# longkaimao/Sentinel

Measured on AMD Instinct MI355X. Metric: flow decisions/sec (node) at 1M flowIds, 1/2/4/8 GPU; HBM GB/s vs peak, higher is better.
Workload: dtype int64; 1 GPU; C3 cluster token server: ClusterFlowChecker, FLOW_THRESHOLD_GLOBAL, S=10/1000 ms; flow_ids=1000000, flow_ids_per_gpu=1000000, parallelism=hash-sharded flowIds x1, rollup=none (1 GPU), namespace_limiter=off

## Files before the change

sentinel_amd/csrc/engine.h:

```cpp
#pragma once

#include <hip/hip_runtime.h>
#include <stddef.h>
#include <stdint.h>

#include "../../include/sentinel_gpu.h"
#include "search_dev.h"

namespace sg {

struct alignas(16) Rule {
    double thr;
    double isec;
    int32_t S;
    int32_t wl;
    int32_t wl_idx;
    int32_t wait_ms;
};
static_assert(sizeof(Rule) == 32, "Rule layout");

struct alignas(64) Bucket {
    int64_t start;
    int64_t c[SG_NUM_EVENTS];
};
static_assert(sizeof(Bucket) == 64, "Bucket layout");

struct alignas(16) BucketHot {
    int64_t start;
    int32_t pass;
    int32_t wait;
};
static_assert(sizeof(BucketHot) == 16, "BucketHot layout");

__device__ __forceinline__ void store_hot(BucketHot* h, int64_t start, int64_t pass, int64_t wait) {
    BucketHot x;
    x.start = start;
    x.pass = (int32_t)pass;
    x.wait = (int32_t)wait;
    *h = x;
}

struct alignas(16) Occ {
    int64_t pass;
    int64_t pass_req;
};

#ifndef SG_SORT_ROUNDS
#define SG_SORT_ROUNDS 16
#endif
constexpr int kSortRounds = SG_SORT_ROUNDS;
constexpr int kMaxWl = 8;
constexpr uint32_t kMaxPeriods = 1u << 16;
constexpr int kShortMax = 256;
constexpr int kLdsBnd = 4096;
constexpr int kLdsBndFlow = 1024;
#ifndef SG_RECW
#define SG_RECW 32
#endif
constexpr int kRecW = SG_RECW;
constexpr int kClasses = 6;
constexpr uint32_t kClassMax[kClasses - 1] = {4, 16, 64, 256, 1024};

constexpr int kErrTime = 1;
constexpr int kErrPeriods = 2;
constexpr int kErrInternal = 16;
constexpr int kErrExchange = 64;

struct BatchArgs {
    const sg_req* req;
    sg_result* out;
    uint64_t n;
    uint64_t* rec;
    uint32_t* hist0;
    uint32_t* csum0;
    int hist0_bits;
    uint64_t* rec_sorted;
    int kshift;
    int abits;
    uint64_t imask;
    uint64_t amask;
    uint64_t aesc;
    uint32_t K;
    const Rule* rules;
    Bucket* ring;
    BucketHot* hot;
    Occ* occ;
    int stride;
    double max_occ_ratio;
    int n_wl;
    int32_t wl[kMaxWl];
    uint32_t* bnd;
    int64_t* p0;
    uint32_t* np;
    int* err;
    int64_t* last_ts;
    int check_last;
    int64_t* front_ts;
    int walk_cus;
    uint32_t* long_list;
    uint32_t* long_count;
    uint32_t* short_list;
    uint32_t* short_count;
    uint32_t* short_key;
    uint32_t* long_key;
    uint32_t* seg_end;
    uint32_t* seg_start;
    uint32_t* short_end;
    uint32_t* long_end;
    int seg_marked;
    uint32_t* long_pend;
    uint64_t class_off[kClasses];
    uint32_t short_max;
    uint32_t* exit_cnt;
    uint64_t exit_amask;
    int dbg;
    int narrow;
    int generic_walker;
    int tiny;
    unsigned long long* dbg_ctr;
    uint4* skips;
    uint32_t* skip_count;
    uint32_t skip_cap;
    int hist0_shift;
    int bin_on;
    int prep_tiles;
    int bin_dshift;
    int bin_bsh;
    uint32_t bin_R;
    uint2* hot_tab;
    uint32_t* hot_key;
    uint64_t* bin_buf;
    const uint32_t* bin_tot;
};

constexpr int kBinDigit = 10;
constexpr uint32_t kBinRegular = 512;
constexpr uint32_t kBinHot = (1u << kBinDigit) - kBinRegular - 1;
constexpr uint32_t kBinDrop = (1u << kBinDigit) - 1;
constexpr int kBinMaxBsh = 11;
constexpr int kHotBucketBits = 9;
constexpr uint32_t kHotWays = 4;
constexpr uint32_t kHotTab = kHotWays << kHotBucketBits;
constexpr uint32_t kHotEmpty = 0xFFFFFFFFu;
__host__ __device__ __forceinline__ uint32_t hot_hash(uint32_t key) {
    return (key * 2654435761u) >> (32 - kHotBucketBits);
}

constexpr int kLongPeriods = 16;
constexpr uint32_t kLongTab = 65536;
constexpr uint32_t kSkipMin = 256;
constexpr uint32_t kSkipPiece = 4096;

constexpr int kMaxLim = 8;
constexpr int kLimSamples = 10;
constexpr int kLimWindowMs = 100;

struct LimRing {
    int64_t start[kLimSamples];
    int64_t count[kLimSamples];
};

static_assert(sizeof(sg_req) % sizeof(int64_t) == 0 && sizeof(sg_cparam_req) % sizeof(int64_t) == 0 &&
                  offsetof(sg_req, ts_ms) == 0 && offsetof(sg_cparam_req, ts_ms) == 0,
              "LimArgs::ts strides over the request records");
struct LimArgs {
    int n_lim;
    int wl_idx;
    double qps[kMaxLim];
    const uint8_t* rule_lim;
    uint8_t* slot;
    uint32_t* tile_tot;
    uint32_t* tile_off;
    uint32_t* arrivals;
    uint32_t* prefix;
    uint32_t* quota;
    LimRing* ring;
    const uint32_t* xg;
    const int64_t* ts;
    uint32_t ts_stride;
    int64_t t_base;
    uint32_t n_ms;
    int world, rank;
};

hipError_t launch_limiter(const BatchArgs& a, const LimArgs& L, hipStream_t stream);
hipError_t launch_limiter_plan_only(const BatchArgs& a, const LimArgs& L, hipStream_t stream);
hipError_t launch_lim_arrivals(const sg_req* req, uint64_t n, uint32_t K, const uint8_t* rule_lim, int64_t t_base,
                               uint32_t n_ms, uint32_t* counts, int* err, hipStream_t stream);
hipError_t launch_lim_arrivals_param(const sg_cparam_req* req, uint64_t n, uint32_t K, const uint8_t* rule_lim,
                                     int64_t t_base, uint32_t n_ms, uint32_t* counts, int* err, hipStream_t stream);

constexpr int kErrNonPositive = 4;
constexpr int kErrTableFull = 8;

struct PRule {
    int64_t token_count;
    int64_t duration_sec;
    int32_t burst;
    int32_t behavior;
    int32_t max_queueing_ms;
    uint32_t hot_begin, hot_count;
    uint32_t pad;
    uint64_t table_base;
    uint64_t table_mask;
};

struct alignas(16) CxSide {
    int64_t t;
    uint32_t psl;
    uint32_t node;
};

struct alignas(32) PSlot {
    uint64_t value;
    uint32_t flags;
    uint32_t pad;
    int64_t time;
    int64_t tokens;
};

constexpr uint32_t kPcBuckets = 2048;

struct PArgs {
    const sg_param_req* req;
    int32_t* out;
    uint64_t n;
    uint64_t* rec;
    uint64_t* rec_sorted;
    int ibits;
    uint64_t imask;
    int gshift;
    uint32_t* msb;
    int64_t* mt0;
    uint32_t* mnp;
    uint16_t* mbk;
    int bshift;
    const PRule* rules;
    uint32_t n_rules;
    const sg_param_hot_item* hot;
    PSlot* table;
    uint64_t total_slots;
    int* err;
    int64_t* last_ts;
    uint32_t* long_list;
    uint32_t* long_count;
    uint32_t short_max;
};

struct alignas(32) PSThread {
    unsigned long long owner;
    uint64_t value;
    int64_t count;
    int64_t pad;
};

hipError_t launch_param_clear(PSlot* table, uint64_t n, hipStream_t stream);
hipError_t launch_param_batch(const PArgs& p, const BatchArgs& sg, uint64_t* a_buf, uint64_t* b_buf, uint32_t* hist,
                              int lo_bit, int hi_bit, uint64_t** sorted_out, hipStream_t stream, hipStream_t aux,
                              hipEvent_t fork, hipEvent_t join);

struct PaceRule {
    double count;
    int32_t max_queueing_ms;
    int32_t pad;
};

struct PaceArgs {
    const sg_pace_req* req;
    int32_t* out;
    uint64_t n;
    uint64_t* rec;
    uint64_t* rec_sorted;
    int ibits;
    uint64_t imask;
    const PaceRule* rules;
    uint32_t n_rules;
    int64_t* latest;
    int* err;
    int64_t* last_ts;
    uint32_t* long_list;
    uint32_t* long_count;
    uint32_t* short_list;
    uint32_t short_max;
    int gshift;
    uint32_t* msb;
    int64_t* mt0;
    uint32_t* mnp;
    uint16_t* mbk;
    int bshift;
    uint64_t class_off[kClasses];
};

hipError_t launch_pace_batch(const PaceArgs& p, uint64_t* a_buf, uint64_t* b_buf, uint32_t* hist, int lo_bit, int hi_bit,
                             uint64_t** sorted_out, hipStream_t stream, hipStream_t aux, hipEvent_t fork,
                             hipEvent_t join);

constexpr int kErrBounds = 32;

struct CPRule {
    double count;
    double isec;
    int32_t S;
    int32_t wl;
    int32_t global;
    int32_t connected;
    uint32_t hot_begin, hot_count;
    uint64_t table_base;
    uint64_t table_mask;
    int32_t wl_idx;
    int32_t pad;
};

struct CPBucket {
    int64_t start;
    int64_t count;
};

struct CPArgs {
    const sg_cparam_req* req;
    const uint64_t* values;
    uint64_t n_values;
    sg_result* out;
    uint64_t n;
    uint64_t* rec;
    int ibits;
    uint64_t imask;
    const CPRule* rules;
    uint32_t n_rules;
    const sg_param_hot_item* hot;
    uint64_t* keys;
    CPBucket* ring;
    int stride;
    uint64_t total_slots;
    uint64_t per;
    int* err;
    int64_t* last_ts;
};

struct CPBatch {
    uint32_t* owner;
    uint8_t* chk;
    uint8_t* assume;
    uint64_t* rec;
    int pbits;
    uint64_t pmask;
    int idbits;
    uint64_t idmask;
    int n_wl;
    int32_t wl[kMaxWl];
    uint32_t* bnd;
    int64_t* p0;
    uint32_t* np;
    int* changed;
    const int* changed_prev;
    CPBucket* save;
    uint32_t* pslot;
    uint32_t* dflag;
    uint32_t* item_start;
    uint32_t* item_end;
    uint32_t* item_slot;
    uint32_t* slot_item;
    uint32_t* din;
    uint32_t* din_count;
    uint32_t* dout;
// ... 574 lines not shown
```

sentinel_amd/csrc/engine.hip:

```cpp
#include "engine.h"

#include <algorithm>
#include <cstdlib>
#include <mutex>

namespace sg {


__device__ __forceinline__ int32_t java_d2i(double x) {
    if (x != x) return 0;
    if (x >= 2147483647.0) return INT32_MAX;
    if (x <= -2147483648.0) return INT32_MIN;
    return (int32_t)x;
}

__device__ __forceinline__ int lane_id() { return (int)__lane_id(); }

__device__ __forceinline__ double qps_of(int64_t sum, double isec) { return avg_div((double)sum, isec); }

__device__ __forceinline__ int64_t wave_sum(int64_t v) {
#pragma unroll
    for (int o = 32; o > 0; o >>= 1) v += __shfl_xor((long long)v, o, 64);
    return v;
}
// ... 1050 lines not shown
    __syncthreads();
    if (diag) tk1 = __builtin_amdgcn_s_memrealtime();
    uint32_t tk[kBinPer], sst[kBinPer], slot[kBinPer], gb = 0;
    if (small) {
        const Cnt16 cnt{lw};
#pragma unroll
        for (int u = 0; u < kBinRows; ++u) {
            const uint32_t j = c0 + (uint32_t)u * 64 + (uint32_t)lane;
            if (j < c1) cnt.inc((uint32_t)wave * kBinKeys + (uint32_t)(v[u] >> a.kshift) - kb0);
        }
        __syncthreads();
        if (diag) tk2 = __builtin_amdgcn_s_memrealtime();
        bin_scan_lists(a, cnt, nk, wsum, lcnt, tk, sst, slot);
        __syncthreads();
        if (tid < kL && lcnt[tid]) gb = atomicAdd(tid == kClasses ? a.long_count : a.short_count + tid, lcnt[tid]);
        if (diag) tk3 = __builtin_amdgcn_s_memrealtime();
        uint32_t pos[kBinRows / 2];
#pragma unroll
        for (int u = 0; u < kBinRows; ++u) {
            const uint32_t j = c0 + (uint32_t)u * 64 + (uint32_t)lane;
            const bool valid = j < c1;
            const uint32_t d = valid ? (uint32_t)(v[u] >> a.kshift) - kb0 : 0u;
            const uint64_t peers = match_key(d) & __ballot(valid);
            const uint32_t ci = (uint32_t)wave * kBinKeys + d;
            const uint32_t c = cnt.get(ci);
            const uint32_t p16 = valid ? c + (uint32_t)__popcll(peers & lt) : 0xFFFFu;
            pos[u / 2] = (u & 1) ? (pos[u / 2] | (p16 << 16)) : p16;
            cnt.set(ci, c + (uint32_t)__popcll(peers));
            __builtin_amdgcn_sched_barrier(0);
        }
        if (diag) tp4 = __builtin_amdgcn_s_memrealtime();
        uint64_t* stage = lds + (kBinWaves * kBinKeys * 2) / 8;
        uint64_t* dst = a.rec_sorted + s0;
        for (uint32_t w0 = 0; w0 < len; w0 += kBinStage) {
#pragma unroll
            for (int u = 0; u < kBinRows; ++u) {
                const uint32_t p = (pos[u / 2] >> ((u & 1) * 16)) & 0xFFFFu;
                if (p != 0xFFFFu && p - w0 < kBinStage) stage[p - w0] = v[u];
            }
            __syncthreads();
            const uint32_t m = min(kBinStage, len - w0);
            for (uint32_t p = tid; p < m; p += kBinThreads) dst[w0 + p] = stage[p];
            __syncthreads();
        }
    } else {
        uint32_t(*cnt)[kBinKeys] = reinterpret_cast<uint32_t(*)[kBinKeys]>(lw);
        struct Cnt32 {
            uint32_t* w;
            __device__ __forceinline__ uint32_t get(uint32_t i) const { return w[i]; }
            __device__ __forceinline__ void set(uint32_t i, uint32_t x) const { w[i] = x; }
        } c32{lw};
        for (uint32_t r0 = c0; r0 < c1; r0 += 64u * kBinRows) {
            if (r0 != c0) {
#pragma unroll
                for (int u = 0; u < kBinRows; ++u) v[u] = src[min(r0 + (uint32_t)u * 64 + (uint32_t)lane, last)];
            }
#pragma unroll
            for (int u = 0; u < kBinRows; ++u) {
                const uint32_t j = r0 + (uint32_t)u * 64 + (uint32_t)lane;
                if (j < c1) atomicAdd(&cnt[wave][(uint32_t)(v[u] >> a.kshift) - kb0], 1u);
            }
        }
        __syncthreads();
        if (diag) tk2 = __builtin_amdgcn_s_memrealtime();
        bin_scan_lists(a, c32, nk, wsum, lcnt, tk, sst, slot);
        __syncthreads();
        if (tid < kL && lcnt[tid]) gb = atomicAdd(tid == kClasses ? a.long_count : a.short_count + tid, lcnt[tid]);
        if (diag) tk3 = __builtin_amdgcn_s_memrealtime();
        uint64_t* dst = a.rec_sorted + s0;
        for (uint32_t r0 = c0; r0 < c1; r0 += 64u * kBinRows) {
#pragma unroll
            for (int u = 0; u < kBinRows; ++u) v[u] = src[min(r0 + (uint32_t)u * 64 + (uint32_t)lane, last)];
#pragma unroll
            for (int u = 0; u < kBinRows; ++u) {
                const uint32_t j = r0 + (uint32_t)u * 64 + (uint32_t)lane;
                const bool valid = j < c1;
                const uint32_t d = valid ? (uint32_t)(v[u] >> a.kshift) - kb0 : 0u;
                const uint64_t peers = match_key(d) & __ballot(valid);
                const uint32_t c = cnt[wave][d];
                if (valid) {
                    dst[c + (uint32_t)__popcll(peers & lt)] = v[u];
                    if (lane == __builtin_ctzll(peers)) cnt[wave][d] = c + (uint32_t)__popcll(peers);
                }
                __builtin_amdgcn_sched_barrier(0);
            }
        }
    }
    if (diag) tp5 = __builtin_amdgcn_s_memrealtime();
    if (tid < kL) lbase[tid] = gb;
    __syncthreads();
    if (diag) tp6 = __builtin_amdgcn_s_memrealtime();
    bin_emit(a, lbase, s0, kb0, tk, sst, slot);
    if (diag) {
        __syncthreads();
        if (tid == 0) {
            const uint64_t tk4 = __builtin_amdgcn_s_memrealtime();
            if (small) {
                atomicAdd(&a.dbg_ctr[48], (unsigned long long)(tp4 - tk3));
                atomicAdd(&a.dbg_ctr[49], (unsigned long long)(tp5 - tp4));
                atomicAdd(&a.dbg_ctr[50], (unsigned long long)(tp6 - tp5));
                atomicAdd(&a.dbg_ctr[51], (unsigned long long)(tk4 - tp6));
            }
            atomicAdd(&a.dbg_ctr[40], (unsigned long long)(tk1 - tk0));
            atomicAdd(&a.dbg_ctr[41], (unsigned long long)(tk2 - tk1));
            atomicAdd(&a.dbg_ctr[42], (unsigned long long)(tk3 - tk2));
            atomicAdd(&a.dbg_ctr[43], (unsigned long long)(tk4 - tk3));
            atomicAdd(&a.dbg_ctr[44], 1ull);
            atomicAdd(&a.dbg_ctr[45], small ? 0ull : 1ull);
            atomicAdd(&a.dbg_ctr[47], (unsigned long long)len);
        }
    }
}

__global__ void __launch_bounds__(1024) k_hot_update(BatchArgs a) {
    __shared__ uint32_t hcnt[32];
    __shared__ uint32_t thr, nslot;
    __shared__ uint32_t tkey[kHotTab], tslot[kHotTab], bfill[kHotTab / kHotWays];
    const uint32_t tid = threadIdx.x;
    if (tid < 32) hcnt[tid] = 0;
    if (tid == 0) nslot = 0;
    for (uint32_t x = tid; x < kHotTab; x += 1024) {
        tkey[x] = kHotEmpty;
        tslot[x] = 0;
    }
    for (uint32_t x = tid; x < kHotTab / kHotWays; x += 1024) bfill[x] = 0;
    __syncthreads();
    const uint32_t nl = *a.err ? 0u : *a.long_count;
    for (uint32_t i = tid; i < nl; i += 1024) {
        const uint32_t len = a.long_end[i] - a.long_list[i];
        atomicAdd(&hcnt[31 - __clz(len)], 1u);
    }
    __syncthreads();
    if (tid == 0) {
        uint32_t cum = 0, t = 0;
        for (int c = 31; c >= 0; --c) {
            cum += hcnt[c];
            if (cum >= kBinHot) {
                t = (uint32_t)c;
                break;
            }
        }
        thr = t;
    }
    __syncthreads();
    for (int pass = 0; pass < 2; ++pass) {
        for (uint32_t i = tid; i < nl; i += 1024) {
            const uint32_t len = a.long_end[i] - a.long_list[i];
            const uint32_t c = 31 - __clz(len);
            if (pass == 0 ? c <= thr : c != thr) continue;
            if (nslot >= kBinHot) continue;
            const uint32_t k = a.long_key[i];
            const uint32_t bk = hot_hash(k);
            const uint32_t w = atomicAdd(&bfill[bk], 1u);
            if (w >= kHotWays) continue;
            const uint32_t s = atomicAdd(&nslot, 1u);
            if (s >= kBinHot) {
                tkey[bk * kHotWays + w] = kHotEmpty;
                continue;
            }
            a.hot_key[s] = k;
            tkey[bk * kHotWays + w] = k;
            tslot[bk * kHotWays + w] = s;
        }
        __syncthreads();
    }
    for (uint32_t x = tid; x < kHotTab; x += 1024) a.hot_tab[x] = make_uint2(tkey[x], tslot[x]);
}

__global__ void __launch_bounds__(256) k_hot_reset(uint2* hot_tab) {
    for (uint32_t x = threadIdx.x; x < kHotTab; x += 256) hot_tab[x] = make_uint2(kHotEmpty, 0u);
}

__device__ __forceinline__ void stage_periods(const BatchArgs& a) {
    uint32_t tot = 0;
    for (int w = 0; w < a.n_wl; ++w) tot += a.np[w];
    const bool lds = tot <= (uint32_t)kLdsBndFlow && !(a.dbg & 1);
    uint32_t off = 0;
    for (int w = 0; w < a.n_wl; ++w) {
        const uint32_t npw = a.np[w];
        if (lds) {
            const uint32_t* g = a.bnd + (size_t)w * kMaxPeriods;
            for (uint32_t i = threadIdx.x; i < npw; i += blockDim.x) g_sbnd[off + i] = g[i];
        }
        if (threadIdx.x == 0) g_boff[w] = off;
        off += npw;
    }
    if (threadIdx.x == 0) g_blds = lds ? 1 : 0;
    if (threadIdx.x < (unsigned)a.n_wl) {
        g_p0[threadIdx.x] = a.p0[threadIdx.x];
        g_np[threadIdx.x] = a.np[threadIdx.x];
    }
    for (uint32_t x = threadIdx.x; x < (uint32_t)a.n_wl * (kModS + 1); x += blockDim.x) {
        const uint32_t w = x / (kModS + 1), m = x % (kModS + 1);
        g_p0mod[w][m] = m ? (uint8_t)(a.p0[w] % (int64_t)m) : (uint8_t)0;
    }
    __syncthreads();
}

template <bool L>
__device__ __forceinline__ void walk_long_body(const BatchArgs& a) {
    const int lane = lane_id();
    const uint32_t n_long = *a.long_count;
    const uint32_t wave = blockIdx.x * (blockDim.x / 64) + threadIdx.x / 64;
    const uint32_t nwaves = gridDim.x * (blockDim.x / 64);
    for (uint32_t item = wave; item < n_long; item += nwaves) {
        const uint64_t s = a.long_list[item];
        uint32_t k;
        uint64_t e;
        if (a.long_key && a.seg_end) {
            k = a.long_key[item];
            e = a.long_end ? a.long_end[item] : a.seg_end[k];
        } else {
            k = (uint32_t)(a.rec_sorted[s] >> a.kshift);
            e = gallop_search(s + (a.short_max ? a.short_max : 1), a.n, [&](uint64_t p) {
                return (uint32_t)(a.rec_sorted[p] >> a.kshift) != k;
            }, lane);
        }
        const uint64_t t0 = (a.dbg & 64) ? __builtin_amdgcn_s_memrealtime() : 0;
        walk_wave<L>(a, k, s, e, item);
        if (a.dbg & 64) {
            const uint64_t t1 = __builtin_amdgcn_s_memrealtime();
            const uint64_t len = e - s;
            const int b = len <= 64 ? 0 : len <= 256 ? 1 : len <= 1024 ? 2 : 3;
            if (lane == 0) {
                atomicAdd(&a.dbg_ctr[16 + 2 * b], 1ull);
                atomicAdd(&a.dbg_ctr[17 + 2 * b], (unsigned long long)(t1 - t0));
                atomicMax(&a.dbg_ctr[24 + b], (unsigned long long)(t1 - t0));
            }
        }
    }
}

__global__ void __launch_bounds__(256) k_long_bounds(BatchArgs a) {
    if (*a.err) return;
    const uint32_t n_long = min(*a.long_count, kLongTab);
    const uint32_t total = n_long * (uint32_t)kLongPeriods;
    for (uint32_t t = blockIdx.x * blockDim.x + threadIdx.x; t < total; t += gridDim.x * blockDim.x) {
        const uint32_t item = t / kLongPeriods, q = t % kLongPeriods;
        const uint32_t k = a.long_key[item];
        const int w = a.rules[k].wl_idx;
        const uint32_t npw = a.np[w];
        if (npw > (uint32_t)kLongPeriods || q + 1 >= npw) continue;
        const uint32_t nb = a.bnd[(size_t)w * kMaxPeriods + q + 1];
        uint64_t lo = a.long_list[item], hi = a.long_end ? a.long_end[item] : a.seg_end[k];
        while (lo < hi) {
            const uint64_t mid = (lo + hi) >> 1;
            if ((uint32_t)((a.rec_sorted[mid] >> a.abits) & a.imask) >= nb) hi = mid;
            else lo = mid + 1;
        }
        a.long_pend[t] = (uint32_t)lo;
    }
}

#ifndef SG_WLONG_BLOCKS
#define SG_WLONG_BLOCKS 2
#endif
__global__ void __launch_bounds__(256, SG_WLONG_BLOCKS) k_walk_long(BatchArgs a) {
    if (*a.err || (a.dbg & 4096)) return;
    stage_periods(a);
    if (g_blds) walk_long_body<true>(a);
    else walk_long_body<false>(a);
}


struct SlotSnap {
    int32_t st, pass, wait;
};
constexpr int32_t kSnapOld = -(1 << 30);

__device__ __forceinline__ int32_t rel32(int64_t x) {
    return x > (int64_t)INT32_MAX ? INT32_MAX : x < (int64_t)INT32_MIN ? INT32_MIN : (int32_t)x;
}

__device__ __forceinline__ int32_t snap_rel(int64_t start, int64_t T0) {
    if (start == INT64_MIN) return INT32_MIN;
    const int64_t d = start - T0;
    return d < (int64_t)kSnapOld ? kSnapOld : d > (int64_t)(1 << 30) ? (1 << 30) : (int32_t)d;
}

__device__ __forceinline__ bool narrow_span(const BatchArgs& a, int64_t T0) {
    bool ok = true;
    for (int w = 0; w < a.n_wl; ++w) {
        const int64_t wl = a.wl[w];
        const int64_t b = a.p0[w] * wl;
        ok = ok && (b + ((int64_t)a.np[w] + 1) * wl - T0 < (1ll << 29)) &&
             (b - ((int64_t)a.stride + 1) * wl - T0 > -(1ll << 29));
    }
    return ok;
}

__device__ __forceinline__ bool tiny_active(const BatchArgs& a) {
    return a.tiny && a.narrow && narrow_span(a, a.p0[0] * (int64_t)a.wl[0]);
}

__device__ __forceinline__ void store_bucket(Bucket* b, BucketHot* h, int64_t start, const int64_t* c) {
    ulonglong2* p = reinterpret_cast<ulonglong2*>(b);
    p[0] = make_ulonglong2((unsigned long long)start, (unsigned long long)c[0]);
    p[1] = make_ulonglong2((unsigned long long)c[1], (unsigned long long)c[2]);
    p[2] = make_ulonglong2((unsigned long long)c[3], (unsigned long long)c[4]);
    p[3] = make_ulonglong2((unsigned long long)c[5], (unsigned long long)c[6]);
    store_hot(h, start, c[SG_EV_PASS], c[SG_EV_WAITING]);
}

constexpr int kBlk = 4;

template <int SM, bool L>
__device__ __forceinline__ void walk_reg(const BatchArgs& a, bool act, uint32_t k, uint64_t s, uint64_t e,
                                         const Rule& R, const Occ& occ, SlotSnap* snap, uint64_t* buf, int64_t T0) {
    Bucket* ring = a.ring + (size_t)k * a.stride;
    BucketHot* hot = a.hot + (size_t)k * a.stride;
    const int S = R.S;
    const int64_t wl = R.wl;
    PeriodCursor<L> pc;
    pc.init(a, act ? R.wl_idx : 0);
    const int64_t P0 = g_p0[act ? R.wl_idx : 0];
    PeriodState ps;
    ps.occ_pass = occ.pass;
    ps.occ_req = occ.pass_req;
#pragma unroll
    for (int ev = 0; ev < SG_NUM_EVENTS; ++ev) ps.cur[ev] = 0;
    ps.wo_pass = ps.wo_wait = ps.head_other = 0;
    int I = -1;
    int64_t ws = 0;
    const uint64_t n1 = a.n - 1;
    uint64_t nb[kBlk];
    uint64_t p = s;
    int left = kBlk;
    bool more = act && p + kBlk < e;
#pragma unroll
    for (int u = 0; u < kBlk; ++u) nb[u] = a.rec_sorted[min(p + kBlk + u, n1)];
    bool live = act;
    uint32_t qn = 0;
    Decoded dn;
    auto peek = [&]() {
        if (p + (uint64_t)(kBlk - left) >= e) {
            live = false;
            return;
        }
        dn = decode(a, buf[0]);
        qn = pc.of(dn.idx);
    };
    auto advance = [&]() {
#pragma unroll
        for (int v = 0; v < kBlk - 1; ++v) buf[v] = buf[v + 1];
        buf[kBlk - 1] = ~0ull;
        if (--left == 0) {
            if (!more) {
                live = false;
                return;
            }
#pragma unroll
            for (int u = 0; u < kBlk; ++u) buf[u] = nb[u];
            p += kBlk;
            left = kBlk;
            more = p + kBlk < e;
#pragma unroll
            for (int u = 0; u < kBlk; ++u) nb[u] = a.rec_sorted[min(p + kBlk + u, n1)];
        }
    };
    if (live) peek();
    while (__ballot(live)) {
        if (live && qn != pc.q) {
            if (I >= 0) {
                if (!(a.dbg & 512)) store_bucket(ring + I, hot + I, ws, ps.cur);
                snap[I].st = (int32_t)(ws - T0);
                snap[I].pass = (int32_t)ps.cur[SG_EV_PASS];
                snap[I].wait = (int32_t)ps.cur[SG_EV_WAITING];
            }
            const uint32_t qprev = pc.q;
            pc.seek(qn);
            const int64_t P = P0 + (int64_t)qn;
            I = I < 0 ? period_slot(R.wl_idx, qn, S) : (int)((uint32_t)(I + (int)(qn - qprev)) % (uint32_t)S);
            ws = P * wl;
            const int64_t lo_rel = ws - (int64_t)S * wl - T0;
            const int32_t lo32 = rel32(lo_rel);
            const int h = I + 1 == S ? 0 : I + 1;
            int32_t sx[SM], px[SM], wx[SM];
#pragma unroll
            for (int x = 0; x < SM; ++x) {
                sx[x] = snap[x].st;
                px[x] = snap[x].pass;
                wx[x] = snap[x].wait;
            }
            uint32_t wp = 0, ww = 0, ho = 0;
#pragma unroll
            for (int x = 0; x < SM; ++x) {
                const bool v = (x < S) & (x != I) & (sx[x] > lo32);
                const uint32_t m = v ? 0xFFFFFFFFu : 0u;
                wp += (uint32_t)px[x] & m;
                ww += (uint32_t)wx[x] & m;
                ho = (x == h) ? ((uint32_t)px[x] & m) : ho;
            }
            ps.wo_pass = (int64_t)wp;
            ps.wo_wait = (int64_t)ww;
            ps.head_other = (int64_t)ho;
            const int32_t stI_rel = snap[I].st;
            const int64_t stI = stI_rel == INT32_MIN ? INT64_MIN : T0 + (int64_t)stI_rel;
            int64_t cI[SG_NUM_EVENTS];
            if (stI == ws) {
#pragma unroll
                for (int ev = 0; ev < SG_NUM_EVENTS; ++ev) cI[ev] = ring[I].c[ev];
            }
            open_bucket(ps, stI, cI, ws);
        }
        while (live && qn == pc.q) {
            const double latest = qps_of(ps.wo_pass + ps.cur[SG_EV_PASS], R.isec);
            const double next_remaining = R.thr - latest - (double)dn.acq;
            if (next_remaining >= 0) {
                ps.cur[SG_EV_PASS] += dn.acq;
                ps.cur[SG_EV_PASS_REQUEST] += 1;
                if (dn.prio) ps.cur[SG_EV_OCCUPIED_PASS] += dn.acq;
                if (!(a.dbg & 256)) store_result(a.out, dn.idx, SG_STATUS_OK, java_d2i(next_remaining), 0);
            } else {
                int32_t wait;
                const int32_t stt = decide_fail(R, a.max_occ_ratio, ps, dn.acq, dn.prio, &wait);
                if (stt != SG_STATUS_BLOCKED && !(a.dbg & 256)) store_result(a.out, dn.idx, stt, 0, wait);
            }
            advance();
            if (live) peek();
        }
    }

    if (act) {
        if (I >= 0) store_bucket(ring + I, hot + I, ws, ps.cur);
        if (ps.occ_pass != occ.pass || ps.occ_req != occ.pass_req) {
            Occ o;
            o.pass = ps.occ_pass;
            o.pass_req = ps.occ_req;
            a.occ[k] = o;
        }
    }
}

__device__ __forceinline__ void wait_vm0() { __builtin_amdgcn_s_waitcnt(0x0F70); }

template <int R>
__device__ __forceinline__ void glds_rows(const uint32_t* src, uint32_t* wrecs) {
    if constexpr (R > 0) {
        glds_rows<R - 1>(src, wrecs);
        __builtin_amdgcn_global_load_lds((const __attribute__((address_space(1))) void*)src,
                                         (__attribute__((address_space(3))) void*)(wrecs + (R - 1) * 64 - 2 * (R - 1)),
                                         4, 8 * (R - 1), 0);
    }
}

template <int R>
__device__ __forceinline__ void stage_records(const BatchArgs& a, uint32_t* wrecs, uint64_t p) {
    glds_rows<R>(reinterpret_cast<const uint32_t*>(a.rec_sorted + p), wrecs);
}

template <int SM, bool L>
__device__ __forceinline__ void walk_lds(const BatchArgs& a, bool act, uint32_t k, uint64_t s, uint64_t e,
                                         const Rule& R, const Occ& occ, SlotSnap* snap, uint32_t* wrecs, int lane,
                                         int64_t T0, int rows) {
    Bucket* ring = a.ring + (size_t)k * a.stride;
    BucketHot* hot = a.hot + (size_t)k * a.stride;
    const int S = R.S;
    const int64_t wl = R.wl;
    PeriodCursor<L> pc;
    pc.init(a, act ? R.wl_idx : 0);
    const int64_t P0 = g_p0[act ? R.wl_idx : 0];
    PeriodState ps;
    ps.occ_pass = occ.pass;
    ps.occ_req = occ.pass_req;
#pragma unroll
    for (int ev = 0; ev < SG_NUM_EVENTS; ++ev) ps.cur[ev] = 0;
    ps.wo_pass = ps.wo_wait = ps.head_other = 0;
    int I = -1;
    int64_t ws = 0;
    uint64_t wb = s;
    uint64_t p = s;
    bool live = act && p < e;
    bool park = false;
    uint32_t win = (uint32_t)rows;
    uint32_t qn = 0;
    Decoded dn;
    auto peek = [&]() {
        if (p >= e) {
            live = false;
            return;
        }
        if (p - wb >= (uint64_t)win) {
            park = true;
            return;
        }
        dn = decode_c(a, wrecs[(uint32_t)(p - wb) * 64 + lane]);
        qn = pc.of(dn.idx);
    };
    if (live) peek();
    for (;;) {
        if (!__ballot(live && !park)) {
            if (!__ballot(live)) break;
            if (park) {
                stage_records<kRecW>(a, wrecs, p);
                wb = p;
                win = kRecW;
            }
            wait_vm0();
            __builtin_amdgcn_wave_barrier();
            if (park) {
                park = false;
                peek();
            }
            continue;
        }
        if (live && !park && qn != pc.q) {
            if (I >= 0) {
                store_bucket(ring + I, hot + I, ws, ps.cur);
                snap[I].st = (int32_t)(ws - T0);
                snap[I].pass = (int32_t)ps.cur[SG_EV_PASS];
                snap[I].wait = (int32_t)ps.cur[SG_EV_WAITING];
            }
            const uint32_t qprev = pc.q;
            pc.seek(qn);
            const int64_t P = P0 + (int64_t)qn;
            I = I < 0 ? period_slot(R.wl_idx, qn, S) : (int)((uint32_t)(I + (int)(qn - qprev)) % (uint32_t)S);
            ws = P * wl;
            const int64_t lo_rel = ws - (int64_t)S * wl - T0;
            const int32_t lo32 = rel32(lo_rel);
            const int h = I + 1 == S ? 0 : I + 1;
            int32_t sx[SM], px[SM], wx[SM];
#pragma unroll
            for (int x = 0; x < SM; ++x) {
                sx[x] = snap[x].st;
                px[x] = snap[x].pass;
                wx[x] = snap[x].wait;
            }
            uint32_t wp = 0, ww = 0, ho = 0;
#pragma unroll
            for (int x = 0; x < SM; ++x) {
                const bool v = (x < S) & (x != I) & (sx[x] > lo32);
                const uint32_t m = v ? 0xFFFFFFFFu : 0u;
                wp += (uint32_t)px[x] & m;
                ww += (uint32_t)wx[x] & m;
                ho = (x == h) ? ((uint32_t)px[x] & m) : ho;
            }
            ps.wo_pass = (int64_t)wp;
            ps.wo_wait = (int64_t)ww;
            ps.head_other = (int64_t)ho;
            const int32_t stI_rel = snap[I].st;
            const int64_t stI = stI_rel == INT32_MIN ? INT64_MIN : T0 + (int64_t)stI_rel;
            int64_t cI[SG_NUM_EVENTS];
            if (stI == ws) {
#pragma unroll
                for (int ev = 0; ev < SG_NUM_EVENTS; ++ev) cI[ev] = ring[I].c[ev];
            }
            open_bucket(ps, stI, cI, ws);
        }
        while (live && !park && qn == pc.q) {
            const double latest = qps_of(ps.wo_pass + ps.cur[SG_EV_PASS], R.isec);
            const double next_remaining = R.thr - latest - (double)dn.acq;
            if (next_remaining >= 0) {
                ps.cur[SG_EV_PASS] += dn.acq;
                ps.cur[SG_EV_PASS_REQUEST] += 1;
                if (dn.prio) ps.cur[SG_EV_OCCUPIED_PASS] += dn.acq;
                store_result(a.out, dn.idx, SG_STATUS_OK, java_d2i(next_remaining), 0);
            } else {
                int32_t wait;
                const int32_t stt = decide_fail(R, a.max_occ_ratio, ps, dn.acq, dn.prio, &wait);
                if (stt != SG_STATUS_BLOCKED) store_result(a.out, dn.idx, stt, 0, wait);
            }
            ++p;
            peek();
        }
    }
    if (act) {
        if (I >= 0) store_bucket(ring + I, hot + I, ws, ps.cur);
        if (ps.occ_pass != occ.pass || ps.occ_req != occ.pass_req) {
            Occ o;
            o.pass = ps.occ_pass;
            o.pass_req = ps.occ_req;
            a.occ[k] = o;
        }
    }
}

constexpr int kGatherMaxS = 10;
#ifndef SG_SHORT_BLOCKS
#define SG_SHORT_BLOCKS 3
#endif
constexpr int kShortBlocksPerCu = SG_SHORT_BLOCKS;

template <int SM, bool L>
__device__ __forceinline__ void walk_short_lds(const BatchArgs& a, SlotSnap* snap_all, uint32_t* recs_all) {
    static_assert(SM > 0, "LDS ring snapshot");
    const int lane = lane_id();
    const bool tiny = tiny_active(a);
    SlotSnap* snap = snap_all + (threadIdx.x / 64) * (64 * SM);
    uint32_t* wrecs = recs_all + (threadIdx.x / 64) * (kRecW * 64);
    uint32_t cnt[kClasses], grp_end[kClasses];
    uint32_t total = 0;
#pragma unroll
    for (int c = kClasses - 1; c >= 0; --c) {
        cnt[c] = (c == 0 && tiny) ? 0u : a.short_count[c];
        total += (cnt[c] + 63) / 64;
        grp_end[c] = total;
    }
    const uint32_t wave = blockIdx.x * (blockDim.x / 64) + threadIdx.x / 64;
    const uint32_t nwaves = gridDim.x * (blockDim.x / 64);
    if (wave >= total) return;
    const int64_t T0 = a.p0[0] * (int64_t)a.wl[0];
    auto desc = [&](uint32_t g, int& c, bool& act, uint32_t& s, uint32_t& k, uint32_t& e) {
        c = kClasses - 1;
        uint32_t g0 = 0;
        while (g >= grp_end[c]) {
            g0 = grp_end[c];
            --c;
        }
        c = __builtin_amdgcn_readfirstlane(c);
        const uint32_t i = (g - g0) * 64 + (uint32_t)lane;
        act = i < cnt[c];
        const uint64_t li = a.class_off[c] + (act ? i : 0u);
        s = a.short_list[li];
        k = a.short_key[li];
        e = a.short_end[li];
    };
    int c_n;
    bool act_n;
    uint32_t s_n, k_n, e_n;
    desc(wave, c_n, act_n, s_n, k_n, e_n);
    for (uint32_t g = wave; g < total; g += nwaves) {
        const uint64_t tw0 = (a.dbg & 64) ? __builtin_amdgcn_s_memrealtime() : 0;
        const int c = c_n;
        const bool act = act_n;
        const uint64_t s = s_n;
        const uint32_t k = k_n;
        const uint64_t e = e_n;
        const Rule R = a.rules[k];
        const Occ occ = a.occ[k];
        static_assert(kRecW >= (int)kClassMax[1], "the first window of class 1 must fit the lane's LDS rows");
        const int rows = c == 0 ? (int)kClassMax[0] : c == 1 ? (int)kClassMax[1] : kRecW;
        if (c == 0) stage_records<kClassMax[0]>(a, wrecs, s);
        else if (c == 1) stage_records<kClassMax[1]>(a, wrecs, s);
        else stage_records<kRecW>(a, wrecs, s);
        desc(min(g + nwaves, total - 1), c_n, act_n, s_n, k_n, e_n);
        {
            constexpr int kT = SM;
            int gl = lane;
            asm volatile("" : "+v"(gl));
            ulonglong2 v[kT];
#pragma unroll
            for (int t = 0; t < kT; ++t) {
                const int pc = t * 64 + gl;
                const int j = pc / kT;
                const int q = pc % kT;
                const uint32_t kj = (uint32_t)__shfl((int)k, j, 64);
                const int qq = q < a.stride ? q : 0;
                v[t] = *reinterpret_cast<const ulonglong2*>(a.hot + (size_t)kj * a.stride + qq);
            }
            __builtin_amdgcn_sched_barrier(0);
#pragma unroll
            for (int t = 0; t < kT; ++t) asm volatile("" ::"v"(v[t].x), "v"(v[t].y));
#pragma unroll
            for (int t = 0; t < kT; ++t) {
                const int pc = t * 64 + gl;
                SlotSnap& d = snap[pc];
                d.st = snap_rel((int64_t)v[t].x, T0);
                d.pass = (int32_t)(uint32_t)v[t].y;
                d.wait = (int32_t)(uint32_t)(v[t].y >> 32);
            }
        }
        wait_vm0();
        __builtin_amdgcn_fence(__ATOMIC_RELEASE, "wavefront");
        __builtin_amdgcn_wave_barrier();
        __builtin_amdgcn_fence(__ATOMIC_ACQUIRE, "wavefront");
        const uint64_t tw1 = (a.dbg & 64) ? __builtin_amdgcn_s_memrealtime() : 0;
        walk_lds<SM, L>(a, act, k, s, e, R, occ, snap + lane * SM, wrecs, lane, T0, rows);
        if (a.dbg & 64) {
            const uint64_t tw2 = __builtin_amdgcn_s_memrealtime();
            if (lane == 0) {
                atomicAdd(&a.dbg_ctr[0], (unsigned long long)(tw2 - tw0));
                atomicAdd(&a.dbg_ctr[1 + c], 1ull);
                atomicAdd(&a.dbg_ctr[7 + c], (unsigned long long)(tw1 - tw0));
                atomicAdd(&a.dbg_ctr[7 + c], (unsigned long long)(tw2 - tw1) << 32);
            }
        }
    }
}

template <int SM, bool L, bool C>
__device__ __forceinline__ void walk_short_body(const BatchArgs& a, SlotSnap* snap_all, uint32_t* recs_all) {
    if constexpr (SM > 0 && C) {
        const int64_t T0 = a.p0[0] * (int64_t)a.wl[0];
        if (a.narrow && narrow_span(a, T0)) {
            walk_short_lds<SM, L>(a, snap_all, recs_all);
            return;
        }
    }
    constexpr int kSnapPerWave = SM > 0 ? 64 * SM : 1;
    const int lane = lane_id();
    const bool tiny = tiny_active(a);
    SlotSnap* snap = snap_all + (threadIdx.x / 64) * kSnapPerWave;
    uint32_t cnt[kClasses], grp_end[kClasses];
    uint32_t total = 0;
#pragma unroll
    for (int c = kClasses - 1; c >= 0; --c) {
        cnt[c] = (c == 0 && tiny) ? 0u : a.short_count[c];
        total += (cnt[c] + 63) / 64;
        grp_end[c] = total;
    }
    const uint32_t wave = blockIdx.x * (blockDim.x / 64) + threadIdx.x / 64;
    const uint32_t nwaves = gridDim.x * (blockDim.x / 64);
    const int64_t T0 = a.p0[0] * (int64_t)a.wl[0];
    const bool snap_ok = SM > 0 && a.narrow && narrow_span(a, T0);
    for (uint32_t g = wave; g < total; g += nwaves) {
        int c = kClasses - 1;
        uint32_t g0 = 0;
        while (g >= grp_end[c]) {
            g0 = grp_end[c];
            --c;
        }
        c = __builtin_amdgcn_readfirstlane(c);
        const uint32_t i = (g - g0) * 64 + (uint32_t)lane;
        const bool act = i < cnt[c];
        if constexpr (SM > 0 && !C) if (snap_ok) {
            const uint64_t tw0 = (a.dbg & 64) ? __builtin_amdgcn_s_memrealtime() : 0;
            const uint64_t li = a.class_off[c] + (act ? i : 0u);
            const uint64_t s = a.short_list[li];
            const uint32_t k = a.short_key[li];
            const uint64_t e = a.short_end ? a.short_end[li] : a.seg_end[k];
            const Rule R = a.rules[k];
            const Occ occ = a.occ[k];
            uint64_t buf[kBlk];
#pragma unroll
            for (int u = 0; u < kBlk; ++u) buf[u] = a.rec_sorted[min(s + u, a.n - 1)];
            {
                constexpr int kT = SM;
                int gl = lane;
                asm volatile("" : "+v"(gl));
                {
                    ulonglong2 v[SM];
#pragma unroll
                    for (int t = 0; t < SM; ++t) {
                        const int pc = t * 64 + gl;
                        const int j = pc / kT;
                        const int q = pc % kT;
                        const uint32_t kj = (uint32_t)__shfl((int)k, j, 64);
                        const int qq = q < a.stride ? q : 0;
                        v[t] = *reinterpret_cast<const ulonglong2*>(a.hot + (size_t)kj * a.stride + qq);
                    }
#pragma unroll
                    for (int t = 0; t < SM; ++t) {
                        SlotSnap& d = snap[t * 64 + gl];
                        d.st = snap_rel((int64_t)v[t].x, T0);
                        d.pass = (int32_t)(uint32_t)v[t].y;
                        d.wait = (int32_t)(uint32_t)(v[t].y >> 32);
                    }
                }
                __builtin_amdgcn_fence(__ATOMIC_RELEASE, "wavefront");
                __builtin_amdgcn_wave_barrier();
                __builtin_amdgcn_fence(__ATOMIC_ACQUIRE, "wavefront");
            }
            const uint64_t tw1 = (a.dbg & 64) ? __builtin_amdgcn_s_memrealtime() : 0;
            walk_reg<SM, L>(a, act, k, s, e, R, occ, snap + lane * SM, buf, T0);
            if (a.dbg & 64) {
                const uint64_t tw2 = __builtin_amdgcn_s_memrealtime();
                if (lane == 0) {
                    atomicAdd(&a.dbg_ctr[0], (unsigned long long)(tw2 - tw0));
                    atomicAdd(&a.dbg_ctr[1 + c], 1ull);
                    atomicAdd(&a.dbg_ctr[7 + c], (unsigned long long)(tw1 - tw0));
                    atomicAdd(&a.dbg_ctr[7 + c], (unsigned long long)(tw2 - tw1) << 32);
                }
            }
            continue;
        }
        if (!act) continue;
        const uint64_t s = a.short_list[a.class_off[c] + i];
        const uint32_t k = (uint32_t)(a.rec_sorted[s] >> a.kshift);
        const uint64_t lim = s + (uint64_t)min(a.short_max, c < kClasses - 1 ? kClassMax[c] : 0xFFFFFFFFu) + 1;
        uint64_t e = s + 1;
        while (e < a.n && e < lim && (uint32_t)(a.rec_sorted[e] >> a.kshift) == k) ++e;
        walk_serial<L>(a, k, s, e);
    }
}

template <int SM, bool C>
#ifndef SG_SHORT_C_BLOCKS
#define SG_SHORT_C_BLOCKS 2
#endif
__global__ void __launch_bounds__(256, C ? SG_SHORT_C_BLOCKS : kShortBlocksPerCu) k_walk_short(BatchArgs a) {
    static_assert(SM <= kGatherMaxS, "LDS budget of the ring snapshot");
    __shared__ SlotSnap snap_all[4 * (SM > 0 ? 64 * SM : 1)];
    __shared__ uint32_t recs_all[SM > 0 && C ? 4 * kRecW * 64 : 1];
    if (*a.err || (a.dbg & 8192)) return;
    stage_periods(a);
    if (g_blds) walk_short_body<SM, true, C>(a, snap_all, recs_all);
    else walk_short_body<SM, false, C>(a, snap_all, recs_all);
}

template <int SM, bool L>
__device__ __forceinline__ void walk_tiny_body(const BatchArgs& a) {
    constexpr int kR = (int)kClassMax[0];
    const uint32_t cnt = a.short_count[0];
    const uint64_t base = a.class_off[0];
    const int64_t T0 = a.p0[0] * (int64_t)a.wl[0];
    for (uint32_t t = blockIdx.x * blockDim.x + threadIdx.x; t < cnt; t += gridDim.x * blockDim.x) {
        const uint64_t s = a.short_list[base + t];
        const uint32_t k = a.short_key[base + t];
        const uint32_t e = a.short_end[base + t];
        const Rule R = a.rules[k];
        const Occ occ = a.occ[k];
        uint64_t r0 = a.rec_sorted[s], r1 = a.rec_sorted[min(s + 1, a.n - 1)];
        uint64_t r2 = a.rec_sorted[min(s + 2, a.n - 1)], r3 = a.rec_sorted[min(s + 3, a.n - 1)];
        static_assert(kR == 4, "four record registers");
        Bucket* ring = a.ring + (size_t)k * a.stride;
        BucketHot* hot = a.hot + (size_t)k * a.stride;
        int32_t st[SM], pa[SM], wa[SM];
#pragma unroll
        for (int x = 0; x < SM; ++x) {
            const int xx = x < R.S ? x : 0;
            const ulonglong2 hv = *reinterpret_cast<const ulonglong2*>(hot + xx);
            st[x] = snap_rel((int64_t)hv.x, T0);
            pa[x] = (int32_t)(uint32_t)hv.y;
            wa[x] = (int32_t)(uint32_t)(hv.y >> 32);
        }
        PeriodCursor<L> pc;
        pc.init(a, R.wl_idx);
        const int64_t P0 = g_p0[R.wl_idx];
        const int S = R.S;
        PeriodState ps;
        ps.occ_pass = occ.pass;
        ps.occ_req = occ.pass_req;
#pragma unroll
        for (int ev = 0; ev < SG_NUM_EVENTS; ++ev) ps.cur[ev] = 0;
        ps.wo_pass = ps.wo_wait = ps.head_other = 0;
        int I = -1;
        int64_t ws = 0;
        const uint32_t m = e - (uint32_t)s;
        for (uint32_t u = 0; u < m; ++u) {
            const Decoded d = decode(a, r0);
            r0 = r1;
            r1 = r2;
            r2 = r3;
            const uint32_t q = pc.of(d.idx);
            if (q != pc.q) {
                if (I >= 0) {
                    store_bucket(ring + I, hot + I, ws, ps.cur);
#pragma unroll
                    for (int x = 0; x < SM; ++x) {
                        st[x] = x == I ? (int32_t)(ws - T0) : st[x];
                        pa[x] = x == I ? (int32_t)ps.cur[SG_EV_PASS] : pa[x];
                        wa[x] = x == I ? (int32_t)ps.cur[SG_EV_WAITING] : wa[x];
                    }
                }
                const uint32_t qprev = pc.q;
                pc.seek(q);
                const int64_t P = P0 + (int64_t)q;
                I = I < 0 ? period_slot(R.wl_idx, q, S) : (int)((uint32_t)(I + (int)(q - qprev)) % (uint32_t)S);
                ws = P * R.wl;
                const int64_t lo_rel = ws - (int64_t)S * R.wl - T0;
                const int32_t lo32 = rel32(lo_rel);
                const int h = I + 1 == S ? 0 : I + 1;
                uint32_t wp = 0, ww = 0, ho = 0;
                int32_t stI_rel = INT32_MIN;
#pragma unroll
                for (int x = 0; x < SM; ++x) {
                    const bool v = (x < S) & (x != I) & (st[x] > lo32);
                    const uint32_t mk = v ? 0xFFFFFFFFu : 0u;
                    wp += (uint32_t)pa[x] & mk;
                    ww += (uint32_t)wa[x] & mk;
                    ho = (x == h) ? ((uint32_t)pa[x] & mk) : ho;
                    stI_rel = x == I ? st[x] : stI_rel;
                }
                ps.wo_pass = (int64_t)wp;
                ps.wo_wait = (int64_t)ww;
                ps.head_other = (int64_t)ho;
                const int64_t stI = stI_rel == INT32_MIN ? INT64_MIN : T0 + (int64_t)stI_rel;
                int64_t cI[SG_NUM_EVENTS];
// ... 379 lines not shown
```

Measured before the change: 22.40 billion decisions/s.

## Fast-path blocked records once a period is saturated

Adds a saturation flag per period: once a request fails and even an acquire of one would exceed the threshold, later non-priority requests below the escalation bound are counted as blocked without the floating-point QPS check or the decide_fail call. In the LDS window walker, runs of up to kSatN plain records are checked and accumulated into the block counters in one step. The goal is to cut per-record work in hot, over-limit flows. It relies on the packed record-code bit layout and adds optional debug counters.

```diff
diff --git a/sentinel_amd/csrc/engine.h b/sentinel_amd/csrc/engine.h
--- a/sentinel_amd/csrc/engine.h
+++ b/sentinel_amd/csrc/engine.h
@@ -60,6 +60,8 @@
 constexpr int kRecW = SG_RECW;
 constexpr int kClasses = 6;
 constexpr uint32_t kClassMax[kClasses - 1] = {4, 16, 64, 256, 1024};
+constexpr int kDbgSatRecords = 14;
+constexpr int kDbgSatRuns = 15;
 
 constexpr int kErrTime = 1;
 constexpr int kErrPeriods = 2;
diff --git a/sentinel_amd/csrc/engine.hip b/sentinel_amd/csrc/engine.hip
--- a/sentinel_amd/csrc/engine.hip
+++ b/sentinel_amd/csrc/engine.hip
@@ -1376,6 +1376,25 @@
     store_hot(h, start, c[SG_EV_PASS], c[SG_EV_WAITING]);
 }
 
+__device__ __forceinline__ bool period_saturated(double thr, double latest) { return !(thr - latest - 1.0 >= 0); }
+
+#ifndef SG_SAT_N
+#define SG_SAT_N 8
+#endif
+constexpr int kSatN = SG_SAT_N;
+
+__device__ __forceinline__ bool sat_plain(uint32_t c, uint32_t next_b) {
+    return ((c >> 8) < next_b) & ((c & 1u) == 0u) & ((c & 0xFEu) != 0xFEu);
+}
+
+__device__ __forceinline__ void sat_counters(const BatchArgs& a, uint32_t rec, uint32_t ent, int lane) {
+    const int64_t r = wave_sum((int64_t)rec), n = wave_sum((int64_t)ent);
+    if (lane == 0 && r) {
+        atomicAdd(&a.dbg_ctr[kDbgSatRecords], (unsigned long long)r);
+        atomicAdd(&a.dbg_ctr[kDbgSatRuns], (unsigned long long)n);
+    }
+}
+
 constexpr int kBlk = 4;
 
 template <int SM, bool L>
@@ -1406,6 +1425,8 @@
     bool live = act;
     uint32_t qn = 0;
     Decoded dn;
+    bool sat = false;
+    bool run = false;
     auto peek = [&]() {
         if (p + (uint64_t)(kBlk - left) >= e) {
             live = false;
@@ -1476,20 +1497,34 @@
                 for (int ev = 0; ev < SG_NUM_EVENTS; ++ev) cI[ev] = ring[I].c[ev];
             }
             open_bucket(ps, stI, cI, ws);
+            sat = false;
+            run = false;
         }
         while (live && qn == pc.q) {
-            const double latest = qps_of(ps.wo_pass + ps.cur[SG_EV_PASS], R.isec);
-            const double next_remaining = R.thr - latest - (double)dn.acq;
-            if (next_remaining >= 0) {
-                ps.cur[SG_EV_PASS] += dn.acq;
-                ps.cur[SG_EV_PASS_REQUEST] += 1;
-                if (dn.prio) ps.cur[SG_EV_OCCUPIED_PASS] += dn.acq;
-                if (!(a.dbg & 256)) store_result(a.out, dn.idx, SG_STATUS_OK, java_d2i(next_remaining), 0);
+            const bool plain = sat && !dn.prio && dn.acq < (int64_t)a.aesc;
+            if (plain) {
+                ps.cur[SG_EV_BLOCK] += dn.acq;
+                ps.cur[SG_EV_BLOCK_REQUEST] += 1;
+                if (a.dbg & 64) {
+                    atomicAdd(&a.dbg_ctr[kDbgSatRecords], 1ull);
+                    if (!run) atomicAdd(&a.dbg_ctr[kDbgSatRuns], 1ull);
+                }
             } else {
-                int32_t wait;
-                const int32_t stt = decide_fail(R, a.max_occ_ratio, ps, dn.acq, dn.prio, &wait);
-                if (stt != SG_STATUS_BLOCKED && !(a.dbg & 256)) store_result(a.out, dn.idx, stt, 0, wait);
-            }
+                const double latest = qps_of(ps.wo_pass + ps.cur[SG_EV_PASS], R.isec);
+                const double next_remaining = R.thr - latest - (double)dn.acq;
+                if (next_remaining >= 0) {
+                    ps.cur[SG_EV_PASS] += dn.acq;
+                    ps.cur[SG_EV_PASS_REQUEST] += 1;
+                    if (dn.prio) ps.cur[SG_EV_OCCUPIED_PASS] += dn.acq;
+                    if (!(a.dbg & 256)) store_result(a.out, dn.idx, SG_STATUS_OK, java_d2i(next_remaining), 0);
+                } else {
+                    int32_t wait;
+                    const int32_t stt = decide_fail(R, a.max_occ_ratio, ps, dn.acq, dn.prio, &wait);
+                    if (stt != SG_STATUS_BLOCKED && !(a.dbg & 256)) store_result(a.out, dn.idx, stt, 0, wait);
+                    sat = period_saturated(R.thr, latest);
+                }
+            }
+            run = plain;
             advance();
             if (live) peek();
         }
@@ -1548,6 +1583,9 @@
     bool park = false;
     uint32_t win = (uint32_t)rows;
     uint32_t qn = 0;
+    bool sat = false;
+    bool run = false;
+    uint32_t d_rec = 0, d_ent = 0;
     Decoded dn;
     auto peek = [&]() {
         if (p >= e) {
@@ -1620,24 +1658,52 @@
                 for (int ev = 0; ev < SG_NUM_EVENTS; ++ev) cI[ev] = ring[I].c[ev];
             }
             open_bucket(ps, stI, cI, ws);
+            sat = false;
+            run = false;
         }
         while (live && !park && qn == pc.q) {
-            const double latest = qps_of(ps.wo_pass + ps.cur[SG_EV_PASS], R.isec);
-            const double next_remaining = R.thr - latest - (double)dn.acq;
-            if (next_remaining >= 0) {
-                ps.cur[SG_EV_PASS] += dn.acq;
-                ps.cur[SG_EV_PASS_REQUEST] += 1;
-                if (dn.prio) ps.cur[SG_EV_OCCUPIED_PASS] += dn.acq;
-                store_result(a.out, dn.idx, SG_STATUS_OK, java_d2i(next_remaining), 0);
-            } else {
-                int32_t wait;
-                const int32_t stt = decide_fail(R, a.max_occ_ratio, ps, dn.acq, dn.prio, &wait);
-                if (stt != SG_STATUS_BLOCKED) store_result(a.out, dn.idx, stt, 0, wait);
-            }
-            ++p;
+            uint32_t took = 0;
+            if (sat) {
+                const uint32_t r0 = (uint32_t)(p - wb);
+                const uint32_t lim = (uint32_t)min((uint64_t)win, e - wb);
+                uint32_t cw[kSatN];
+#pragma unroll
+                for (int u = 0; u < kSatN; ++u) cw[u] = wrecs[min(r0 + (uint32_t)u, (uint32_t)(kRecW - 1)) * 64 + lane];
+                bool go = true;
+                uint32_t blk = 0;
+#pragma unroll
+                for (int u = 0; u < kSatN; ++u) {
+                    go = go && r0 + (uint32_t)u < lim && sat_plain(cw[u], pc.next_b);
+                    blk += go ? (cw[u] >> 1) & 127u : 0u;
+                    took += go ? 1u : 0u;
+                }
+                ps.cur[SG_EV_BLOCK] += (int64_t)blk;
+                ps.cur[SG_EV_BLOCK_REQUEST] += (int64_t)took;
+                d_rec += took;
+                d_ent += took && !run ? 1u : 0u;
+            }
+            run = took != 0;
+            if (!took) {
+                const double latest = qps_of(ps.wo_pass + ps.cur[SG_EV_PASS], R.isec);
+                const double next_remaining = R.thr - latest - (double)dn.acq;
+                if (next_remaining >= 0) {
+                    ps.cur[SG_EV_PASS] += dn.acq;
+                    ps.cur[SG_EV_PASS_REQUEST] += 1;
+                    if (dn.prio) ps.cur[SG_EV_OCCUPIED_PASS] += dn.acq;
+                    store_result(a.out, dn.idx, SG_STATUS_OK, java_d2i(next_remaining), 0);
+                } else {
+                    int32_t wait;
+                    const int32_t stt = decide_fail(R, a.max_occ_ratio, ps, dn.acq, dn.prio, &wait);
+                    if (stt != SG_STATUS_BLOCKED) store_result(a.out, dn.idx, stt, 0, wait);
+                    sat = period_saturated(R.thr, latest);
+                }
+                took = 1;
+            }
+            p += took;
             peek();
         }
     }
+    if (a.dbg & 64) sat_counters(a, d_rec, d_ent, lane);
     if (act) {
         if (I >= 0) store_bucket(ring + I, hot + I, ws, ps.cur);
         if (ps.occ_pass != occ.pass || ps.occ_req != occ.pass_req) {
```

Measured after the change: 22.74 billion decisions/s (median of 6 runs). 1.5% higher.
